# blacksnail789521/IMM-TSF

Hardware: AMD Instinct MI355X
Metric: forecast windows/sec (train fwd+bwd) on ragged 64-entity batch (higher is better)
Workload: dtype bf16

## Files before the change

### imm-tsf_amd/csrc/ttcn.hip

```cpp
#include "ttcn.hpp"
#include "../../include/immtsf.h"
#include "block_util.hpp"
#include "rowops.hpp"

int g_immtsf_ttcn_fused = 1;

namespace {

constexpr int LC = 32;

struct Dims { int P, L, F, K, NC, Fp, Kp, NCp, R; };
inline int r4(int x) { return (x + 31) / 32 * 32; }
inline Dims mk_dims(int P, int L, int te_dim, int K) {
    Dims d;
    d.P = P; d.L = L; d.F = 1 + te_dim; d.K = K; d.NC = d.F * K;
    d.Fp = r4(d.F); d.Kp = r4(K); d.NCp = r4(d.NC); d.R = P * L;
    return d;
}

__global__ __launch_bounds__(256) void build_x_kernel(Dims d, const float* __restrict__ x, const float* __restrict__ tt,
                                                       const float* ws, const float* bs, const float* __restrict__ wp,
                                                       const float* __restrict__ bp, float* __restrict__ X) {
    const long idx = (long)blockIdx.x * 256 + threadIdx.x;
    if (idx >= (long)d.R * d.Fp) return;
// ... 91 lines not shown
    const float* mp = mask + (size_t)p * d.L;
    for (int l0 = 0; l0 < d.L; l0 += LC) {
        const int lcnt = min(LC, d.L - l0);
        if (col) {
            for (int l = 0; l < lcnt; ++l) {
                const float smd = Sp[(size_t)(l0 + l) * d.NCp] * dpk;
                smt[l * d.NC + c] = smd;
                Sp[(size_t)(l0 + l) * d.NCp] = smd * (Xp[(size_t)(l0 + l) * d.Fp + fc] - ct) * mp[l0 + l];
            }
        }
        __syncthreads();
        for (int i = c; i < lcnt * d.Fp; i += nt) {
            const int l = i / d.Fp, f = i % d.Fp;
            float a = 0.f;
            if (f < d.F) for (int k = 0; k < d.K; ++k) a += smt[l * d.NC + k * d.F + f];
            dX[((size_t)p * d.L + l0 + l) * d.Fp + f] = a;
        }
        __syncthreads();
    }
}

struct Ws {
    float *X, *h1, *h2, *S, *ctr, *W1p, *b1p, *W2p, *b2p, *W3p, *b3p, *pack;
    size_t bytes;
};
Ws carve_ws(const Dims& d, void* base) {
    Carver k(base);
    Ws w;
    w.X = k.take<float>((size_t)d.R * d.Fp);
    w.h1 = k.take<float>((size_t)d.R * d.Kp);
    w.h2 = k.take<float>((size_t)d.R * d.Kp);
    w.S = k.take<float>((size_t)d.R * d.NCp);
    w.ctr = k.take<float>((size_t)d.P * (d.NC > d.F * 32 ? d.NC : d.F * 32));
    w.W1p = k.take<float>(d.Kp * d.Fp);
    w.b1p = k.take<float>(d.Kp);
    w.W2p = k.take<float>(d.Kp * d.Kp);
    w.b2p = k.take<float>(d.Kp);
    w.W3p = k.take<float>((size_t)d.NCp * d.Kp);
    w.b3p = k.take<float>(d.NCp);
    w.pack = k.take<float>(ttcn_full_pack_floats(d.F));
    w.bytes = k.bytes();
    return w;
}
struct Sc {
    float *dX, *dpool, *dz2, *dz1, *gW1p, *gb1p, *gW2p, *gb2p, *gW3p, *gb3p, *red, *slab;
    size_t bytes;
};
Sc carve_sc(const Dims& d, void* base) {
    Carver k(base);
    Sc s;
    s.dX = k.take<float>((size_t)d.R * d.Fp);
    s.dpool = k.take<float>((size_t)d.P * d.K);
    s.dz2 = k.take<float>((size_t)d.R * d.Kp);
    s.dz1 = k.take<float>((size_t)d.R * d.Kp);
    s.gW1p = k.take<float>(d.Kp * d.Fp);
    s.gb1p = k.take<float>(d.Kp);
    s.gW2p = k.take<float>(d.Kp * d.Kp);
    s.gb2p = k.take<float>(d.Kp);
    s.gW3p = k.take<float>((size_t)d.NCp * d.Kp);
    s.gb3p = k.take<float>(d.NCp);
    s.red = k.take<float>(64 * (d.NCp + 64) + 2 * 256 * d.F);
    s.slab = k.take<float>(ttcn_full_slab_floats(d.F));
    s.bytes = k.bytes();
// ... 33 lines not shown
int immtsf_patch_flatten3(const float* x, const float* tt, const float* mask, int32_t B, int32_t M, int32_t L, int32_t N, float* ox,
                          float* ott, float* omask, immtsf_stream_t stream) {
    if (!x || !tt || !mask || !ox || !ott || !omask || B < 0 || M <= 0 || L <= 0 || N <= 0) return IMMTSF_EINVAL;
    const size_t total = (size_t)B * M * L * N;
    if (total == 0) return IMMTSF_OK;
    hipLaunchKernelGGL(patch_flatten3_kernel, dim3((unsigned)((total + 255) / 256)), dim3(256), 0, static_cast<hipStream_t>(stream), x, tt, mask,
                       B, M, L, N, ox, ott, omask);
    IMMTSF_LAUNCH_CHECK();
    return IMMTSF_OK;
}

int immtsf_ttcn_forward(int32_t P, int32_t L, int32_t te_dim, int32_t ttcn_dim, int32_t precision, const float* x,
                        const float* tt, const float* mask, const immtsf_ttcn_params* p, float* out, int32_t out_ld,
                        int32_t flag_col, void* workspace, size_t workspace_bytes, immtsf_stream_t stream) {
    if (!x || !tt || !mask || !p || !out || !workspace) return IMMTSF_EINVAL;
    if (out_ld < ttcn_dim || flag_col >= out_ld || (flag_col >= 0 && flag_col < ttcn_dim)) return IMMTSF_EINVAL;
    if (bad_dims(P, L, te_dim, ttcn_dim)) return (1 + te_dim) * ttcn_dim > 1024 ? IMMTSF_EUNSUPPORTED : IMMTSF_EINVAL;
    if (P == 0) return IMMTSF_OK;
    const Dims d = mk_dims(P, L, te_dim, ttcn_dim);
    Ws w = carve_ws(d, workspace);
    if (workspace_bytes < w.bytes) return IMMTSF_EWORKSPACE;
    hipStream_t s = static_cast<hipStream_t>(stream);
    if (g_immtsf_ttcn_fused && ttcn_full_supported(precision, L, d.F, d.K))
        return launch_ttcn_full_fwd(P, L, d.F, d.K, x, tt, mask, p, w.pack, w.ctr, out, out_ld, flag_col, s);
    PackPtrs q{p->W1, p->b1, p->W2, p->b2, p->W3, p->b3, w.W1p, w.b1p, w.W2p, w.b2p, w.W3p, w.b3p};
    hipLaunchKernelGGL(pack_w_kernel, dim3(cdiv(d.NCp * d.Kp, 256)), dim3(256), 0, s, d, q);
    IMMTSF_LAUNCH_CHECK();
    const long nx = (long)d.R * d.Fp;
    hipLaunchKernelGGL(build_x_kernel, dim3((unsigned)((nx + 255) / 256)), dim3(256), 0, s, d, x, tt, p->te_scale_w, p->te_scale_b,
                       p->te_per_w, p->te_per_b, w.X);
    IMMTSF_LAUNCH_CHECK();
    {
        GemmArgs g = gemm_args(d.R, d.Kp, d.Fp, d.Fp, d.Fp, d.Kp);
        set_problem(g, 0, w.X, w.W1p, w.h1, w.b1p);
        g.act = 1;
        CHECK(immtsf_launch_gemm(GEMM_NT, precision, g, s));
    }
    {
        GemmArgs g = gemm_args(d.R, d.Kp, d.Kp, d.Kp, d.Kp, d.Kp);
        set_problem(g, 0, w.h1, w.W2p, w.h2, w.b2p);
        g.act = 1;
        CHECK(immtsf_launch_gemm(GEMM_NT, precision, g, s));
    }
    {
        GemmArgs g = gemm_args(d.R, d.NCp, d.Kp, d.Kp, d.Kp, d.NCp);
        set_problem(g, 0, w.h2, w.W3p, w.S, w.b3p);
        CHECK(immtsf_launch_gemm(GEMM_NT, precision, g, s));
    }
    const int threads = cdiv(d.NC, 64) * 64;
    hipLaunchKernelGGL(pool_fwd_kernel, dim3(P), dim3(threads), d.NC * sizeof(float), s, d, w.S, w.X, mask, p->T_bias, w.ctr, out, out_ld, flag_col);
    IMMTSF_LAUNCH_CHECK();
    return IMMTSF_OK;
}

int immtsf_ttcn_backward(int32_t P, int32_t L, int32_t te_dim, int32_t ttcn_dim, int32_t precision, const float* x,
                         const float* tt, const float* mask, const immtsf_ttcn_params* p, const float* out,
                         const float* dout, int32_t out_ld, void* workspace, size_t workspace_bytes, void* scratch,
                         size_t scratch_bytes, const immtsf_ttcn_params* gr, int32_t te_accumulate, immtsf_stream_t stream) {
    if (!tt || !mask || !p || !out || !dout || !gr || !workspace || !scratch || out_ld < ttcn_dim) return IMMTSF_EINVAL;
    if (bad_dims(P, L, te_dim, ttcn_dim)) return IMMTSF_EINVAL;
    if (P == 0) return IMMTSF_OK;
    const Dims d = mk_dims(P, L, te_dim, ttcn_dim);
    Ws w = carve_ws(d, workspace);
    Sc sc = carve_sc(d, scratch);
    if (workspace_bytes < w.bytes || scratch_bytes < sc.bytes) return IMMTSF_EWORKSPACE;
    hipStream_t s = static_cast<hipStream_t>(stream);
    if (g_immtsf_ttcn_fused && ttcn_full_supported(precision, L, d.F, d.K))
        return launch_ttcn_full_bwd(P, L, d.F, d.K, x, tt, mask, p, w.pack, w.ctr, out, dout, out_ld, sc.slab, gr,
                                    static_cast<hipStream_t>(stream), te_accumulate);
    {
        const size_t nbytes = (size_t)((char*)(sc.gb3p + d.NCp) - (char*)sc.gW1p);
        if (int rc = launch_fill(sc.gW1p, 0.f, nbytes / sizeof(float), s)) return rc;
    }
    Fork fk(s);
    {
        const int threads = cdiv(d.NC, 64) * 64;
        const size_t lds = (size_t)(d.K + LC * d.NC) * sizeof(float);
        if (lds > 160 * 1024) return IMMTSF_EUNSUPPORTED;
        hipLaunchKernelGGL(pool_bwd_kernel, dim3(P), dim3(threads), lds, s, d, w.S, w.X, mask, w.ctr, out, dout, out_ld, sc.dX, sc.dpool);
        IMMTSF_LAUNCH_CHECK();
    }
    CHECK(launch_colsum(sc.dpool, nullptr, P, nullptr, d.K, d.K, gr->T_bias, 0, sc.red, s));
    {
        GemmArgs h = gemm_args(d.NCp, d.Kp, d.R, d.NCp, d.Kp, d.Kp);
        set_problem(h, 0, w.S, w.h2, sc.gW3p, nullptr, sc.gb3p);
        h.c_prezeroed = 1;
        CHECK(immtsf_launch_gemm(GEMM_TN, precision, h, fk.fork()));
        GemmArgs g = gemm_args(d.R, d.Kp, d.NCp, d.NCp, d.Kp, d.Kp);
        set_problem(g, 0, w.S, w.W3p, sc.dz2, nullptr);
        g.relu_ref = w.h2; g.ld_ref = d.Kp;
        CHECK(immtsf_launch_gemm(GEMM_NN, precision, g, s));
// ... 31 lines not shown
```

### imm-tsf_amd/csrc/ttcn.hpp

```cpp
#pragma once
#include "common.hpp"

struct immtsf_ttcn_params;
bool ttcn_full_supported(int precision, int L, int F, int K);
size_t ttcn_full_pack_floats(int F);
size_t ttcn_full_slab_floats(int F);
int launch_ttcn_full_fwd(int P, int L, int F, int K, const float* x, const float* tt, const float* mask, const immtsf_ttcn_params* p,
                         float* pack, float* ctr, float* out, int out_ld, int flag_col, hipStream_t s);
int launch_ttcn_full_bwd(int P, int L, int F, int K, const float* x, const float* tt, const float* mask, const immtsf_ttcn_params* p,
                         const float* pack, const float* ctr, const float* out, const float* dout, int out_ld, float* slab,
                         const immtsf_ttcn_params* gr, hipStream_t s, int te_acc = 0);
```

### imm-tsf_amd/csrc/ttcn_full.hip

```cpp
#include "ttcn.hpp"
#include "../../include/immtsf.h"
#include "common.hpp"
#include <stdio.h>
#include <stdlib.h>

int g_immtsf_ttcn_bwd_grid = 0;

namespace {

typedef short s16x8 __attribute__((ext_vector_type(8)));
typedef float f32x2 __attribute__((ext_vector_type(2)));

constexpr int KP = 32;
constexpr int PT = 40;


struct FD { int P, L, F, K, NCq, dbg; };

struct Slab { int W1, b1, W2, b2, W3, b3, te, Tb, total; };
__host__ __device__ inline Slab slab_of(int F) {
    Slab s;
    int o = 0;
    s.W1 = o; o += KP * KP;
    s.b1 = o; o += KP;
    s.W2 = o; o += KP * KP;
    s.b2 = o; o += KP;
    s.W3 = o; o += F * 32 * KP;
    s.b3 = o; o += F * 32;
    s.te = o; o += 2 * KP;
    s.Tb = o; o += KP;
    s.total = o;
    return s;
}

__device__ __forceinline__ bf16x8 load8_bf16(const float* __restrict__ src) {
    const float4 a = *reinterpret_cast<const float4*>(src), b = *reinterpret_cast<const float4*>(src + 4);
    bf16x8 r;
    r[0] = (bf16_t)a.x; r[1] = (bf16_t)a.y; r[2] = (bf16_t)a.z; r[3] = (bf16_t)a.w;
    r[4] = (bf16_t)b.x; r[5] = (bf16_t)b.y; r[6] = (bf16_t)b.z; r[7] = (bf16_t)b.w;
    return r;
}
__device__ __forceinline__ float col_sum(float v) { return xor32_sum(xor16_sum(v)); }
__device__ __forceinline__ float col_max(float v) { return xor32_max(xor16_max(v)); }
__device__ __forceinline__ float row_sum16(float v) { return row16_sum(v); }
__device__ __forceinline__ bf16x8 frag_row(const bf16_t* tile, int pitch, int row0, int k0, int fr, int fq) {
    return *reinterpret_cast<const bf16x8*>(tile + (row0 + fr) * pitch + k0 + fq * 8);
}
__device__ __forceinline__ bf16x8 frag_kmajor(const bf16_t* tile, int pitch, int rbase, int kbase, int fr, int fq) {
    typedef __attribute__((address_space(3))) s16x4 lds_s16x4;
    const int q = fr >> 2, pp = fr & 3;
    const bf16_t* a0 = tile + (kbase + fq * 8 + q) * pitch + rbase + 4 * pp;
    const s16x4 lo = __builtin_amdgcn_ds_read_tr16_b64_v4i16((lds_s16x4*)(a0));
    const s16x4 hi = __builtin_amdgcn_ds_read_tr16_b64_v4i16((lds_s16x4*)(a0 + 4 * pitch));
    const s16x8 v = __builtin_shufflevector(lo, hi, 0, 1, 2, 3, 4, 5, 6, 7);
    return __builtin_bit_cast(bf16x8, v);
}
__device__ __forceinline__ f32x4 mfma(bf16x8 a, bf16x8 b, f32x4 c) { return __builtin_amdgcn_mfma_f32_16x16x32_bf16(a, b, c, 0, 0, 0); }
__device__ __forceinline__ f32x4 zero4() { return f32x4{0.f, 0.f, 0.f, 0.f}; }

struct TEp { const float *ws, *bs, *wp, *bp; };

template <int RT, bool BWD>
struct PatchIn {
    static constexpr int ROWS = RT * 16, HEAD = 3 * ROWS + (BWD ? KP : 0);
    float row, c[2];
    __device__ __forceinline__ void fetch(const FD& d, int p, const float* __restrict__ x, const float* __restrict__ tt,
                                          const float* __restrict__ mask, const float* __restrict__ ctr, const float* __restrict__ out,
                                          const float* __restrict__ dout, int out_ld) {
        const int tid = threadIdx.x;
        row = 0.f; c[0] = c[1] = 0.f;
        if (tid < 3 * ROWS) {
            const int which = tid / ROWS, l = tid % ROWS;
            if (l < d.L) row = (which == 0 ? tt : which == 1 ? x : mask)[(size_t)p * d.L + l];
        } else if (BWD && tid < HEAD) {
            const int k = tid - 3 * ROWS;
            if (k < d.K) row = out[(size_t)p * out_ld + k] > 0.f ? dout[(size_t)p * out_ld + k] : 0.f;
        }
        if (BWD) {
#pragma unroll
            for (int j = 0; j < 2; ++j) {
                const int i = tid + 256 * j;
                if (i < d.NCq) c[j] = ctr[(size_t)p * d.NCq + i];
            }
        }
    }
    __device__ __forceinline__ void park(const FD& d, float* blk) const {
        const int tid = threadIdx.x;
        if (tid < HEAD) blk[tid] = row;
        if (BWD) {
#pragma unroll
            for (int j = 0; j < 2; ++j) {
                const int i = tid + 256 * j;
                if (i < d.NCq) blk[HEAD + i] = c[j];
            }
        }
    }
};

struct XCol { float w, b; int kind; };
__device__ __forceinline__ XCol x_col(const FD& d, TEp te) {
    const int f = threadIdx.x & 31;
    XCol c{0.f, 0.f, 3};
    if (f == 0) c.kind = 0;
    else if (f == 1) { c.w = te.ws[0]; c.b = te.bs[0]; c.kind = 1; }
    else if (f < d.F) { c.w = te.wp[f - 2]; c.b = te.bp[f - 2]; c.kind = 2; }
    return c;
}

template <int RT> constexpr int xt_pitch() { return RT * 16 + 4; }
template <int RT, bool TR = false>
__device__ __forceinline__ void build_x(const FD& d, const XCol xc, const float* blk, bf16_t* Xb, float* Xf, float* Xc = nullptr) {
    const int f = threadIdx.x & 31;
#pragma unroll
    for (int j = 0; j < RT * 2; ++j) {
        const int l = (threadIdx.x >> 5) + 8 * j;
        float v = 0.f, c = 0.f, t = 0.f;
        if (l < d.L && xc.kind != 3) {
            t = blk[l];
            if (xc.kind == 0) v = blk[RT * 16 + l];
            else {
                const float ph = fmaf(xc.w, t, xc.b);
// ... 17 lines not shown
        const int rt = t >> 1, nt = t & 1;
        const f32x4 acc = mfma(frag_row(in, PT, rt * 16, 0, fr, fq), load8_bf16(W + (nt * 16 + fr) * KP + fq * 8), zero4());
        const float bias = b[nt * 16 + fr];
#pragma unroll
        for (int r = 0; r < 4; ++r) outp[(rt * 16 + fq * 4 + r) * PT + nt * 16 + fr] = (bf16_t)fmaxf(acc[r] + bias, 0.f);
    }
}

template <int RT>
__device__ __forceinline__ void mlp_layer_frag(const bf16_t* in, bf16_t* outp, const bf16x8 wf, const float bias, int wave, int fr, int fq) {
    for (int t = wave; t < RT * 2; t += 4) {
        const int rt = t >> 1, nt = t & 1;
        const f32x4 acc = mfma(frag_row(in, PT, rt * 16, 0, fr, fq), wf, zero4());
#pragma unroll
        for (int r = 0; r < 4; ++r) outp[(rt * 16 + fq * 4 + r) * PT + nt * 16 + fr] = (bf16_t)fmaxf(acc[r] + bias, 0.f);
    }
}

struct Wts { const float *W1p, *b1p, *W2p, *b2p, *W3q, *b3q; };

template <int RT, int MF>
__global__ __launch_bounds__(256) void ttcn_full_fwd_kernel(FD d, const float* __restrict__ x, const float* __restrict__ tt,
                                                             const float* __restrict__ mask, TEp te, Wts w, const bf16_t* __restrict__ W3h,
                                                             const float* __restrict__ Tb, float* __restrict__ ctr,
                                                             float* __restrict__ out, int out_ld, int flag_col) {
    extern __shared__ __attribute__((aligned(16))) unsigned char smem[];
    constexpr int ROWS = RT * 16, XP = xt_pitch<RT>();
    constexpr float LOG2E = 1.4426950408889634f;
    bf16_t* Xb = reinterpret_cast<bf16_t*>(smem);
    bf16_t* h1s = Xb + ROWS * PT;
    bf16_t* h2s = h1s + ROWS * PT;
    float* Xf = reinterpret_cast<float*>(h2s + ROWS * PT);
    float* cl = Xf + 16 * XP;
    float* pin = cl + d.NCq;
    const int tid = threadIdx.x, lane = tid & 63, wave = tid >> 6, fr = lane & 15, fq = lane >> 4;
    bf16x8 bw[MF][2];
    float b3v[MF][2];
    const int tnt = wave & 1;
    typedef PatchIn<RT, false> PI;
    PI nx;
    nx.fetch(d, blockIdx.x, x, tt, mask, nullptr, nullptr, nullptr, 0);
    const XCol xc = x_col(d, te);
    const bf16x8 mw1 = load8_bf16(w.W1p + (tnt * 16 + fr) * KP + fq * 8), mw2 = load8_bf16(w.W2p + (tnt * 16 + fr) * KP + fq * 8);
    const float mb1 = w.b1p[tnt * 16 + fr], mb2 = w.b2p[tnt * 16 + fr];
    const float tb = tid < d.K ? Tb[tid] : 0.f;
#pragma unroll
    for (int j = 0; j < MF; ++j)
#pragma unroll
        for (int half = 0; half < 2; ++half) {
            const int f = wave + 4 * j, c = f * 32 + half * 16 + fr;
            bw[j][half] = bf16x8{0, 0, 0, 0, 0, 0, 0, 0};
            b3v[j][half] = 0.f;
            if (f < d.F) { bw[j][half] = *reinterpret_cast<const bf16x8*>(W3h + (size_t)c * KP + fq * 8); b3v[j][half] = w.b3q[c] * LOG2E; }
        }
    nx.park(d, pin);
    __syncthreads();
    int it = 0;
    for (int p = blockIdx.x; p < d.P; p += gridDim.x, ++it) {
    const float* cur = pin + (it & 1) * PI::HEAD;
    const int pn = p + gridDim.x;
    if (pn < d.P) nx.fetch(d, pn, x, tt, mask, nullptr, nullptr, nullptr, 0);
    build_x<RT, true>(d, xc, cur, Xb, Xf);
    __syncthreads();
    mlp_layer_frag<RT>(Xb, h1s, mw1, mb1, wave, fr, fq);
    __syncthreads();
    mlp_layer_frag<RT>(h1s, h2s, mw2, mb2, wave, fr, fq);
    __syncthreads();
    bf16x8 a[RT];
    bool on[RT][4];
    float cval[RT][4];
#pragma unroll
    for (int rt = 0; rt < RT; ++rt) {
        a[rt] = frag_row(h2s, PT, rt * 16, 0, fr, fq);
        const f32x4 m4 = *reinterpret_cast<const f32x4*>(cur + 2 * ROWS + rt * 16 + fq * 4);
#pragma unroll
        for (int r = 0; r < 4; ++r) {
            on[rt][r] = m4[r] != 0.f;
            cval[rt][r] = rt * 16 + fq * 4 + r < d.L ? -1e8f * LOG2E : -INFINITY;
        }
    }
#pragma unroll
    for (int j = 0; j < MF; ++j) {
        const int f = wave + 4 * j;
        if (f < d.F) {
// ... 23 lines not shown
                            m = fmaxf(m, v[rt][h][e]);
                        }
                }
                m = col_max(m);
                f32x2 s2{0.f, 0.f}, p2{0.f, 0.f};
#pragma unroll
                for (int rt = 0; rt < RT; ++rt)
#pragma unroll
                    for (int h = 0; h < 2; ++h) {
                        v[rt][h] -= m;
                        v[rt][h][0] = __builtin_amdgcn_exp2f(v[rt][h][0]);
                        v[rt][h][1] = __builtin_amdgcn_exp2f(v[rt][h][1]);
                        s2 += v[rt][h];
                        p2 += v[rt][h] * xf[rt][h];
                    }
                const float acc = col_sum(p2[0] + p2[1]) * __builtin_amdgcn_rcpf(col_sum(s2[0] + s2[1]));
                if (fq == 0) {
                    cl[c] = acc;
                    ctr[(size_t)p * d.NCq + c] = acc;
                }
            }
        }
    }
    if (pn < d.P) nx.park(d, pin + ((it + 1) & 1) * PI::HEAD);
    __syncthreads();
    if (tid < d.K) {
        float s = tb;
        for (int f = 0; f < d.F; ++f) s += cl[f * 32 + tid];
        out[(size_t)p * out_ld + tid] = fmaxf(s, 0.f);
    }
    if (flag_col >= 0 && wave == 1) {
        float any = lane < d.L ? cur[2 * ROWS + lane] : 0.f;
        any = wave_sum(any);
        if (lane == 0) out[(size_t)p * out_ld + flag_col] = any > 0.f ? 1.f : 0.f;
    }
    __syncthreads();
    }
}

struct WtsT { const bf16_t *W3T , *W2T , *W1T , *W3h ; };

template <int RT, int MF>
__global__ __launch_bounds__(256) __attribute__((amdgpu_waves_per_eu(RT == 2 ? 2 : 1))) void ttcn_full_bwd_kernel(FD d, const float* __restrict__ x, const float* __restrict__ tt,
                                                             const float* __restrict__ mask, TEp te, Wts w, WtsT wt,
                                                             const float* __restrict__ ctr, const float* __restrict__ out,
                                                             const float* __restrict__ dout, int out_ld, float* __restrict__ slab) {
    extern __shared__ __attribute__((aligned(16))) unsigned char smem[];
    constexpr int ROWS = RT * 16, PTT = ROWS + 8, XP = xt_pitch<RT>();
    constexpr float LOG2E = 1.4426950408889634f;
    bf16_t* Xb = reinterpret_cast<bf16_t*>(smem);
    bf16_t* h1s = Xb + ROWS * PT;
    bf16_t* h2s = h1s + ROWS * PT;
    bf16_t* dz2s = h2s + ROWS * PT;
    bf16_t* dz1s = h2s;
    bf16_t* dST = dz2s + ROWS * PT;
    float* Xf = reinterpret_cast<float*>(dST + d.NCq * PTT);
    float* Xc = Xf + 16 * XP;
    typedef PatchIn<RT, true> PI;
    const int PIN = PI::HEAD + d.NCq;
    float* pin = Xc + 16 * XP;
    bf16_t* W3s = reinterpret_cast<bf16_t*>(pin + 2 * PIN);
    bf16_t* W1s = W3s + d.NCq * PT;
    bf16_t* W2s = W1s + KP * PT;
    float* b3s = reinterpret_cast<float*>(W2s + KP * PT);
    const int tid = threadIdx.x, lane = tid & 63, wave = tid >> 6, fr = lane & 15, fq = lane >> 4;
    const Slab sl = slab_of(d.F);
    PI nx;
    nx.fetch(d, blockIdx.x, x, tt, mask, ctr, out, dout, out_ld);
    const XCol xc = x_col(d, te);
    for (int i = tid; i < d.NCq * 4; i += 256) {
        const int c = i >> 2, q = i & 3;
        *reinterpret_cast<bf16x8*>(W3s + c * PT + q * 8) = *reinterpret_cast<const bf16x8*>(wt.W3h + (size_t)c * KP + q * 8);
    }
    for (int i = tid; i < d.NCq; i += 256) b3s[i] = w.b3q[i] * LOG2E;
    if (tid < 2 * KP * 4) {
        const int which = tid >> 7, r = (tid >> 2) & 31, q = tid & 3;
        *reinterpret_cast<bf16x8*>((which ? W2s : W1s) + r * PT + q * 8) = load8_bf16((which ? w.W2p : w.W1p) + r * KP + q * 8);
    }

    f32x4 accW3[MF][2][2];
    f32x2 accB3[MF][2];
#pragma unroll
    for (int j = 0; j < MF; ++j)
#pragma unroll
        for (int half = 0; half < 2; ++half) {
            accW3[j][half][0] = zero4(); accW3[j][half][1] = zero4();
            accB3[j][half] = f32x2{0.f, 0.f};
        }
    const int tnt = wave & 1, tmt = wave >> 1;
    const float mb1 = w.b1p[tnt * 16 + fr], mb2 = w.b2p[tnt * 16 + fr];
    f32x4 accW2 = zero4(), accW1 = zero4();
    float sb2 = 0.f, sb1 = 0.f;
    float accT = 0.f;
    float te_w = 0.f, te_b = 0.f;
    f32x2 tpw[MF], tpb[MF];
#pragma unroll
    for (int j = 0; j < MF; ++j) tpw[j] = tpb[j] = f32x2{0.f, 0.f};

    nx.park(d, pin);
    __syncthreads();
    int it = 0;
    for (int p = blockIdx.x; p < d.P; p += gridDim.x, ++it) {
        const float* cur = pin + (it & 1) * PIN;
        const float *dp = cur + 3 * ROWS, *cts = cur + PI::HEAD;
        const int pn = p + gridDim.x;
        if (pn < d.P) nx.fetch(d, pn, x, tt, mask, ctr, out, dout, out_ld);
        build_x<RT, true>(d, xc, cur, Xb, Xf, Xc);
        __syncthreads();
        if (tid >= 128 && tid < 128 + KP) accT += dp[tid - 128];
        mlp_layer_frag<RT>(Xb, h1s, frag_row(W1s, PT, tnt * 16, 0, fr, fq), mb1, wave, fr, fq);
        __syncthreads();
        mlp_layer_frag<RT>(h1s, h2s, frag_row(W2s, PT, tnt * 16, 0, fr, fq), mb2, wave, fr, fq);
        __syncthreads();
        bf16x8 a[RT];
        bool on[RT][4];
        float cval[RT][4], anyf = 0.f;
        f32x4 t4[RT];
#pragma unroll
        for (int rt = 0; rt < RT; ++rt) {
            a[rt] = frag_row(h2s, PT, rt * 16, 0, fr, fq);
            t4[rt] = *reinterpret_cast<const f32x4*>(cur + rt * 16 + fq * 4);
            const f32x4 m4 = *reinterpret_cast<const f32x4*>(cur + 2 * ROWS + rt * 16 + fq * 4);
#pragma unroll
            for (int r = 0; r < 4; ++r) {
                on[rt][r] = m4[r] != 0.f;
                cval[rt][r] = rt * 16 + fq * 4 + r < d.L ? -1e8f * LOG2E : -INFINITY;
                anyf += on[rt][r] ? 1.f : 0.f;
            }
        }
// ... 108 lines not shown
                const int o = (rt * 16 + fq * 4 + r) * PT + tnt * 16 + fr;
                const float g = (float)h1s[o] > 0.f ? acc[r] : 0.f;
                dz1s[o] = (bf16_t)g;
                sb1 += g;
            }
        }
        __syncthreads();
        if (wave < 2) {
#pragma unroll
            for (int kk = 0; kk < ROWS; kk += 32)
                accW1 = mfma(frag_kmajor(dz1s, PT, wave * 16, kk, fr, fq), frag_kmajor(Xb, PT, 0, kk, fr, fq), accW1);
        }
        for (int rt = (RT == 2 ? wave - 2 : wave); rt >= 0 && rt < RT; rt += 4) {
            const f32x4 acc = mfma(frag_row(dz1s, PT, rt * 16, 0, fr, fq), frag_kmajor(W1s, PT, 0, 0, fr, fq), zero4());
            const f32x4 c4 = *reinterpret_cast<const f32x4*>(Xc + fr * XP + rt * 16 + fq * 4);
            const f32x4 tr = *reinterpret_cast<const f32x4*>(cur + rt * 16 + fq * 4);
#pragma unroll
            for (int r = 0; r < 4; ++r) {
                const float g = acc[r] * c4[r];
                te_w = fmaf(g, tr[r], te_w);
                te_b += g;
            }
        }
        if (pn < d.P) nx.park(d, pin + ((it + 1) & 1) * PIN);
        __syncthreads();
    }

    float* my = slab + (size_t)blockIdx.x * sl.total;
#pragma unroll
    for (int j = 0; j < MF; ++j) {
        const int f = wave + 4 * j;
        if (f < d.F) {
#pragma unroll
            for (int half = 0; half < 2; ++half) {
#pragma unroll
                for (int nt = 0; nt < 2; ++nt)
#pragma unroll
                    for (int r = 0; r < 4; ++r)
                        my[sl.W3 + (size_t)(f * 32 + half * 16 + fq * 4 + r) * KP + nt * 16 + fr] = accW3[j][half][nt][r];
                const float b3sum = col_sum(accB3[j][half][0] + accB3[j][half][1]);
                if (fq == 0) my[sl.b3 + f * 32 + half * 16 + fr] = b3sum;
            }
        }
    }
#pragma unroll
    for (int r = 0; r < 4; ++r) {
        my[sl.W2 + (tmt * 16 + fq * 4 + r) * KP + tnt * 16 + fr] = accW2[r];
        if (wave < 2) my[sl.W1 + (wave * 16 + fq * 4 + r) * KP + fr] = accW1[r];
    }
    if (tid >= 128 && tid < 128 + KP) my[sl.Tb + tid - 128] = accT;
    float* tes = pin;
    if (tid < 4 * KP) tes[tid] = 0.f;
    __syncthreads();
#pragma unroll
    for (int j = 0; j < MF; ++j) {
        const int f = wave + 4 * j;
        const float sw = col_sum(row_sum16(tpw[j][0] + tpw[j][1])), sb = col_sum(row_sum16(tpb[j][0] + tpb[j][1]));
        if (lane == 0 && f >= 1 && f < d.F) {
            atomicAdd(tes + f, sw);
            atomicAdd(tes + KP + f, sb);
        }
    }
    te_w = col_sum(te_w);
    te_b = col_sum(te_b);
    sb2 = col_sum(sb2);
    sb1 = col_sum(sb1);
    if (fq == 0) {
        if (RT == 4 || wave >= 2) {
            atomicAdd(tes + fr, te_w);
            atomicAdd(tes + KP + fr, te_b);
        }
        atomicAdd(tes + 2 * KP + tnt * 16 + fr, sb2);
        atomicAdd(tes + 3 * KP + tnt * 16 + fr, sb1);
    }
    __syncthreads();
    if (tid < 2 * KP) my[sl.te + tid] = tes[tid];
    else if (tid < 3 * KP) my[sl.b2 + tid - 2 * KP] = tes[tid];
    else if (tid < 4 * KP) my[sl.b1 + tid - 3 * KP] = tes[tid];
}

struct PackIn { const float *W1, *b1, *W2, *b2, *W3, *b3; };
__global__ __launch_bounds__(256) void ttcn_pack_kernel(int F, int K, PackIn q, float* W1p, float* b1p, float* W2p, float* b2p,
                                                         float* W3q, float* b3q, bf16_t* W3T, bf16_t* W2T, bf16_t* W1T, bf16_t* W3h) {
    const int i = blockIdx.x * 256 + threadIdx.x, NCq = F * 32;
    if (i < KP * KP) {
        const int r = i >> 5, c = i & 31;
        const float v1 = (r < K && c < F) ? q.W1[r * F + c] : 0.f, v2 = (r < K && c < K) ? q.W2[r * K + c] : 0.f;
        W1p[i] = v1;
        W2p[i] = v2;
        W1T[c * KP + r] = (bf16_t)v1;
        W2T[c * KP + r] = (bf16_t)v2;
    }
    if (i < KP) { b1p[i] = i < K ? q.b1[i] : 0.f; b2p[i] = i < K ? q.b2[i] : 0.f; }
    if (i < NCq * KP) {
        const int c = i >> 5, kk = i & 31, f = c >> 5, k = c & 31;
        const float v = (k < K && kk < K) ? q.W3[(size_t)(k * F + f) * K + kk] : 0.f;
        W3q[i] = v;
        W3T[(size_t)kk * NCq + c] = (bf16_t)v;
        W3h[i] = (bf16_t)v;
    }
    if (i < NCq) { const int f = i >> 5, k = i & 31; b3q[i] = k < K ? q.b3[k * F + f] : 0.f; }
}

struct UnpackOut { float *W1, *b1, *W2, *b2, *W3, *b3, *ws, *bs, *wp, *bp, *Tb; };
__global__ __launch_bounds__(256) void ttcn_unpack_kernel(int F, int K, const float* __restrict__ slab, int nslab, UnpackOut g, int te_acc) {
    __shared__ float red[8][33];
// ... 10 lines not shown
    else if ((i -= n) < K) { dst = g.b1 + i; off = sl.b1 + i; }
    else if ((i -= K) < K) { dst = g.b2 + i; off = sl.b2 + i; }
    else if ((i -= K) < K) { dst = g.Tb + i; off = sl.Tb + i; }
    else if ((i -= K) < 1) { dst = g.ws; off = sl.te + 1; acc = te_acc != 0; }
    else if ((i -= 1) < 1) { dst = g.bs; off = sl.te + KP + 1; acc = te_acc != 0; }
    else if ((i -= 1) < F - 2) { dst = g.wp + i; off = sl.te + 2 + i; acc = te_acc != 0; }
    else if ((i -= F - 2) < F - 2) { dst = g.bp + i; off = sl.te + KP + 2 + i; acc = te_acc != 0; }
    float s = 0.f;
    if (dst) {
#pragma unroll 8
        for (int w = part; w < nslab; w += 8) s += slab[(size_t)w * sl.total + off];
    }
    red[part][slot] = s;
    __syncthreads();
    if (part == 0 && dst) {
#pragma unroll
        for (int q = 1; q < 8; ++q) s += red[q][slot];
        *dst = (acc ? *dst : 0.f) + s;
    }
}
inline int ttcn_unpack_outputs(int F, int K) { return K * F + K * K + F * K * K + F * K + 3 * K + 2 + 2 * (F - 2); }
constexpr int kMaxBwdGrid = 512;

size_t fwd_lds(int RT, int NCq) { return (size_t)RT * 16 * PT * 2 * 3 + (size_t)16 * (RT * 16 + 4) * 4 + (size_t)NCq * 4 + (size_t)2 * 3 * RT * 16 * 4 + 64; }
size_t bwd_lds(int RT, int NCq) {
    const size_t ROWS = RT * 16;
    return ROWS * PT * 2 * 4 + (size_t)NCq * (ROWS + 8) * 2 + 16 * (ROWS + 4) * 4 * 2 + 2 * (3 * ROWS + KP + (size_t)NCq) * 4 + (size_t)(NCq + 2 * KP) * PT * 2 + (size_t)NCq * 4;
}

struct PackPtrs { float *W1p, *b1p, *W2p, *b2p, *W3q, *b3q; bf16_t *W3T, *W2T, *W1T, *W3h; };
PackPtrs pack_ptrs(float* base, int F) {
    PackPtrs q;
    float* o = base;
    q.W1p = o; o += KP * KP;
    q.W2p = o; o += KP * KP;
    q.b1p = o; o += KP;
    q.b2p = o; o += KP;
    q.W3q = o; o += (size_t)F * 32 * KP;
    q.b3q = o; o += F * 32;
    q.W3T = reinterpret_cast<bf16_t*>(o); o += (size_t)F * 32 * KP / 2;
    q.W2T = reinterpret_cast<bf16_t*>(o); o += KP * KP / 2;
    q.W1T = reinterpret_cast<bf16_t*>(o); o += KP * KP / 2;
    q.W3h = reinterpret_cast<bf16_t*>(o);
    return q;
}

}

bool ttcn_full_supported(int precision, int L, int F, int K) {
    return precision == 1 && K >= 1 && K <= 32 && F >= 2 && F <= 16 && L >= 1 && L <= 64;
}
size_t ttcn_full_pack_floats(int F) { return (size_t)2 * KP * KP + 2 * KP + (size_t)F * 32 * KP + F * 32 + (size_t)F * 32 * KP + KP * KP + 64; }
size_t ttcn_full_slab_floats(int F) { return (size_t)kMaxBwdGrid * slab_of(F).total; }

int launch_ttcn_full_fwd(int P, int L, int F, int K, const float* x, const float* tt, const float* mask, const immtsf_ttcn_params* p,
                         float* pack, float* ctr, float* out, int out_ld, int flag_col, hipStream_t s) {
    const FD d{P, L, F, K, F * 32};
    const PackPtrs q = pack_ptrs(pack, F);
    hipLaunchKernelGGL(ttcn_pack_kernel, dim3(cdiv(F * 32 * KP, 256)), dim3(256), 0, s, F, K, PackIn{p->W1, p->b1, p->W2, p->b2, p->W3, p->b3},
                       q.W1p, q.b1p, q.W2p, q.b2p, q.W3q, q.b3q, q.W3T, q.W2T, q.W1T, q.W3h);
    IMMTSF_LAUNCH_CHECK();
    const TEp te{p->te_scale_w, p->te_scale_b, p->te_per_w, p->te_per_b};
    const Wts w{q.W1p, q.b1p, q.W2p, q.b2p, q.W3q, q.b3q};
    const int mf = (F + 3) / 4;
#define TTCN_FWD(RT, MF)                                                                                                                     \
    hipLaunchKernelGGL((ttcn_full_fwd_kernel<RT, MF>), dim3(P < 2048 ? P : 2048), dim3(256), fwd_lds(RT, d.NCq), s, d, x, tt, mask, te, w, q.W3h, p->T_bias, ctr, \
                       out, out_ld, flag_col)
    if (L <= 32) {
        if (mf == 1) TTCN_FWD(2, 1); else if (mf == 2) TTCN_FWD(2, 2); else if (mf == 3) TTCN_FWD(2, 3); else TTCN_FWD(2, 4);
    } else {
        if (mf == 1) TTCN_FWD(4, 1); else if (mf == 2) TTCN_FWD(4, 2); else if (mf == 3) TTCN_FWD(4, 3); else TTCN_FWD(4, 4);
    }
#undef TTCN_FWD
    IMMTSF_LAUNCH_CHECK();
    return IMMTSF_OK;
}

int launch_ttcn_full_bwd(int P, int L, int F, int K, const float* x, const float* tt, const float* mask, const immtsf_ttcn_params* p,
                         const float* pack, const float* ctr, const float* out, const float* dout, int out_ld, float* slab,
                         const immtsf_ttcn_params* gr, hipStream_t s, int te_acc) {
    const FD d{P, L, F, K, F * 32, 0};
    const PackPtrs q = pack_ptrs(const_cast<float*>(pack), F);
    const TEp te{p->te_scale_w, p->te_scale_b, p->te_per_w, p->te_per_b};
    const Wts w{q.W1p, q.b1p, q.W2p, q.b2p, q.W3q, q.b3q};
    const WtsT wt{q.W3T, q.W2T, q.W1T, q.W3h};
    const int genv = g_immtsf_ttcn_bwd_grid;
    int gmax = genv > 0 ? genv : (L <= 32 ? (P >= 8192 ? 512 : 384) : 224);
    gmax = gmax > kMaxBwdGrid ? kMaxBwdGrid : gmax;
    const int grid = P < gmax ? P : gmax;
    const size_t lds = bwd_lds(L <= 32 ? 2 : 4, d.NCq);
    const int mf = (F + 3) / 4;
#define TTCN_BWD(RT, MF)                                                                                                                  \
    do {                                                                                                                                  \
        if (lds > 64 * 1024)                                                                                                              \
            (void)hipFuncSetAttribute(reinterpret_cast<const void*>(ttcn_full_bwd_kernel<RT, MF>), hipFuncAttributeMaxDynamicSharedMemorySize, \
                                      (int)lds);                                                                                          \
        hipLaunchKernelGGL((ttcn_full_bwd_kernel<RT, MF>), dim3(grid), dim3(256), lds, s, d, x, tt, mask, te, w, wt, ctr, out, dout, out_ld, \
                           slab);                                                                                                         \
    } while (0)
    if (L <= 32) {
        if (mf == 1) TTCN_BWD(2, 1); else if (mf == 2) TTCN_BWD(2, 2); else if (mf == 3) TTCN_BWD(2, 3); else TTCN_BWD(2, 4);
    } else {
        if (mf == 1) TTCN_BWD(4, 1); else if (mf == 2) TTCN_BWD(4, 2); else if (mf == 3) TTCN_BWD(4, 3); else TTCN_BWD(4, 4);
    }
#undef TTCN_BWD
    IMMTSF_LAUNCH_CHECK();
    hipLaunchKernelGGL(ttcn_unpack_kernel, dim3(cdiv(ttcn_unpack_outputs(F, K), 32)), dim3(256), 0, s, F, K, slab, grid,
                       UnpackOut{gr->W1, gr->b1, gr->W2, gr->b2, gr->W3, gr->b3, gr->te_scale_w, gr->te_scale_b, gr->te_per_w, gr->te_per_b,
                                 gr->T_bias}, te_acc);
    IMMTSF_LAUNCH_CHECK();
    return IMMTSF_OK;
}
```

Baseline: 157,500.

## Partition TTCN patches into live and empty lists, fast-path fully-masked patches

Adds an ordering pass, fused into the weight-pack kernel plus an optional scatter kernel for large P, that classifies each patch as live or empty (all-zero mask) and writes a compacted index list. The forward and backward fused kernels walk this list, skipping the MLP and GEMM work for empty patches. Forward computes only the mean-based outputs for them; backward handles them in a separate cheap loop that accumulates only the time-embedding gradients. It also swaps some shared-memory atomics for per-wave staging and a deterministic sum. This costs an extra mask scan and more complex control flow, and could pay off on ragged batches with many empty patches.

```diff
diff --git a/imm-tsf_amd/csrc/ttcn.hip b/imm-tsf_amd/csrc/ttcn.hip
--- a/imm-tsf_amd/csrc/ttcn.hip
+++ b/imm-tsf_amd/csrc/ttcn.hip
@@ -137,6 +137,7 @@
 
 struct Ws {
     float *X, *h1, *h2, *S, *ctr, *W1p, *b1p, *W2p, *b2p, *W3p, *b3p, *pack;
+    int* order;
     size_t bytes;
 };
 Ws carve_ws(const Dims& d, void* base) {
@@ -154,6 +155,7 @@
     w.W3p = k.take<float>((size_t)d.NCp * d.Kp);
     w.b3p = k.take<float>(d.NCp);
     w.pack = k.take<float>(ttcn_full_pack_floats(d.F));
+    w.order = k.take<int>(ttcn_full_order_ints(d.P));
     w.bytes = k.bytes();
     return w;
 }
@@ -233,7 +235,7 @@
     if (workspace_bytes < w.bytes) return IMMTSF_EWORKSPACE;
     hipStream_t s = static_cast<hipStream_t>(stream);
     if (g_immtsf_ttcn_fused && ttcn_full_supported(precision, L, d.F, d.K))
-        return launch_ttcn_full_fwd(P, L, d.F, d.K, x, tt, mask, p, w.pack, w.ctr, out, out_ld, flag_col, s);
+        return launch_ttcn_full_fwd(P, L, d.F, d.K, x, tt, mask, p, w.pack, w.order, w.ctr, out, out_ld, flag_col, s);
     PackPtrs q{p->W1, p->b1, p->W2, p->b2, p->W3, p->b3, w.W1p, w.b1p, w.W2p, w.b2p, w.W3p, w.b3p};
     hipLaunchKernelGGL(pack_w_kernel, dim3(cdiv(d.NCp * d.Kp, 256)), dim3(256), 0, s, d, q);
     IMMTSF_LAUNCH_CHECK();
@@ -277,7 +279,7 @@
     if (workspace_bytes < w.bytes || scratch_bytes < sc.bytes) return IMMTSF_EWORKSPACE;
     hipStream_t s = static_cast<hipStream_t>(stream);
     if (g_immtsf_ttcn_fused && ttcn_full_supported(precision, L, d.F, d.K))
-        return launch_ttcn_full_bwd(P, L, d.F, d.K, x, tt, mask, p, w.pack, w.ctr, out, dout, out_ld, sc.slab, gr,
+        return launch_ttcn_full_bwd(P, L, d.F, d.K, x, tt, mask, p, w.pack, w.order, w.ctr, out, dout, out_ld, sc.slab, gr,
                                     static_cast<hipStream_t>(stream), te_accumulate);
     {
         const size_t nbytes = (size_t)((char*)(sc.gb3p + d.NCp) - (char*)sc.gW1p);
diff --git a/imm-tsf_amd/csrc/ttcn.hpp b/imm-tsf_amd/csrc/ttcn.hpp
--- a/imm-tsf_amd/csrc/ttcn.hpp
+++ b/imm-tsf_amd/csrc/ttcn.hpp
@@ -5,8 +5,9 @@
 bool ttcn_full_supported(int precision, int L, int F, int K);
 size_t ttcn_full_pack_floats(int F);
 size_t ttcn_full_slab_floats(int F);
+size_t ttcn_full_order_ints(int P);
 int launch_ttcn_full_fwd(int P, int L, int F, int K, const float* x, const float* tt, const float* mask, const immtsf_ttcn_params* p,
-                         float* pack, float* ctr, float* out, int out_ld, int flag_col, hipStream_t s);
+                         float* pack, int* order, float* ctr, float* out, int out_ld, int flag_col, hipStream_t s);
 int launch_ttcn_full_bwd(int P, int L, int F, int K, const float* x, const float* tt, const float* mask, const immtsf_ttcn_params* p,
-                         const float* pack, const float* ctr, const float* out, const float* dout, int out_ld, float* slab,
-                         const immtsf_ttcn_params* gr, hipStream_t s, int te_acc = 0);
+                         const float* pack, const int* order, const float* ctr, const float* out, const float* dout, int out_ld,
+                         float* slab, const immtsf_ttcn_params* gr, hipStream_t s, int te_acc = 0);
diff --git a/imm-tsf_amd/csrc/ttcn_full.hip b/imm-tsf_amd/csrc/ttcn_full.hip
--- a/imm-tsf_amd/csrc/ttcn_full.hip
+++ b/imm-tsf_amd/csrc/ttcn_full.hip
@@ -16,6 +16,9 @@
 
 
 struct FD { int P, L, F, K, NCq, dbg; };
+
+constexpr int kOrdLive = 0, kOrdList = 4;
+constexpr int kOrdOneWg = 8192, kOrdChunk = 1024;
 
 struct Slab { int W1, b1, W2, b2, W3, b3, te, Tb, total; };
 __host__ __device__ inline Slab slab_of(int F) {
@@ -59,6 +62,16 @@
 __device__ __forceinline__ f32x4 zero4() { return f32x4{0.f, 0.f, 0.f, 0.f}; }
 
 struct TEp { const float *ws, *bs, *wp, *bp; };
+__device__ __forceinline__ void stage_te(const FD& d, TEp te, float* tes) {
+    const int f = threadIdx.x;
+    if (f < 16) {
+        float w = 0.f, b = 0.f;
+        if (f == 1) { w = te.ws[0]; b = te.bs[0]; }
+        else if (f >= 2 && f < d.F) { w = te.wp[f - 2]; b = te.bp[f - 2]; }
+        tes[f] = w;
+        tes[16 + f] = b;
+    }
+}
 
 template <int RT, bool BWD>
 struct PatchIn {
@@ -97,6 +110,23 @@
     }
 };
 
+template <int RT>
+__device__ __forceinline__ float fetch_empty(const FD& d, int p, const float* __restrict__ tt, const float* __restrict__ out,
+                                             const float* __restrict__ dout, int out_ld) {
+    constexpr int ROWS = RT * 16;
+    const int tid = threadIdx.x, k = tid - 3 * ROWS;
+    float v = 0.f;
+    if (tid < ROWS) { if (tid < d.L) v = tt[(size_t)p * d.L + tid]; }
+    else if (k >= 0 && k < d.K) v = out[(size_t)p * out_ld + k] > 0.f ? dout[(size_t)p * out_ld + k] : 0.f;
+    return v;
+}
+template <int RT>
+__device__ __forceinline__ void park_empty(float* blk, float v) {
+    constexpr int ROWS = RT * 16;
+    const int tid = threadIdx.x;
+    if (tid < ROWS || (tid >= 3 * ROWS && tid < 3 * ROWS + KP)) blk[tid] = v;
+}
+
 struct XCol { float w, b; int kind; };
 __device__ __forceinline__ XCol x_col(const FD& d, TEp te) {
     const int f = threadIdx.x & 31;
@@ -160,8 +190,8 @@
 template <int RT, int MF>
 __global__ __launch_bounds__(256) void ttcn_full_fwd_kernel(FD d, const float* __restrict__ x, const float* __restrict__ tt,
                                                              const float* __restrict__ mask, TEp te, Wts w, const bf16_t* __restrict__ W3h,
-                                                             const float* __restrict__ Tb, float* __restrict__ ctr,
-                                                             float* __restrict__ out, int out_ld, int flag_col) {
+                                                             const float* __restrict__ Tb, const int* __restrict__ ord,
+                                                             float* __restrict__ ctr, float* __restrict__ out, int out_ld, int flag_col) {
     extern __shared__ __attribute__((aligned(16))) unsigned char smem[];
     constexpr int ROWS = RT * 16, XP = xt_pitch<RT>();
     constexpr float LOG2E = 1.4426950408889634f;
@@ -171,14 +201,20 @@
     float* Xf = reinterpret_cast<float*>(h2s + ROWS * PT);
     float* cl = Xf + 16 * XP;
     float* pin = cl + d.NCq;
+    float* tes = pin + 2 * 3 * ROWS;
     const int tid = threadIdx.x, lane = tid & 63, wave = tid >> 6, fr = lane & 15, fq = lane >> 4;
+    const int n_live = ord[kOrdLive];
+    const int* __restrict__ list = ord + kOrdList;
+    const int grid = gridDim.x;
+    int p = list[blockIdx.x], pn = blockIdx.x + grid < d.P ? list[blockIdx.x + grid] : -1;
     bf16x8 bw[MF][2];
     float b3v[MF][2];
     const int tnt = wave & 1;
     typedef PatchIn<RT, false> PI;
     PI nx;
-    nx.fetch(d, blockIdx.x, x, tt, mask, nullptr, nullptr, nullptr, 0);
+    nx.fetch(d, p, x, tt, mask, nullptr, nullptr, nullptr, 0);
     const XCol xc = x_col(d, te);
+    stage_te(d, te, tes);
     const bf16x8 mw1 = load8_bf16(w.W1p + (tnt * 16 + fr) * KP + fq * 8), mw2 = load8_bf16(w.W2p + (tnt * 16 + fr) * KP + fq * 8);
     const float mb1 = w.b1p[tnt * 16 + fr], mb2 = w.b2p[tnt * 16 + fr];
     const float tb = tid < d.K ? Tb[tid] : 0.f;
@@ -194,10 +230,29 @@
     nx.park(d, pin);
     __syncthreads();
     int it = 0;
-    for (int p = blockIdx.x; p < d.P; p += gridDim.x, ++it) {
+    for (int i = blockIdx.x; i < d.P; i += grid, ++it) {
     const float* cur = pin + (it & 1) * PI::HEAD;
-    const int pn = p + gridDim.x;
-    if (pn < d.P) nx.fetch(d, pn, x, tt, mask, nullptr, nullptr, nullptr, 0);
+    const int pnn = i + 2 * grid < d.P ? list[i + 2 * grid] : -1;
+    if (pn >= 0) nx.fetch(d, pn, x, tt, mask, nullptr, nullptr, nullptr, 0);
+    if (i >= n_live) {
+        const float invL = __builtin_amdgcn_rcpf((float)d.L);
+#pragma unroll
+        for (int j = 0; j < MF; ++j) {
+            const int f = wave + 4 * j;
+            if (f < d.F) {
+                float v = 0.f;
+                if (lane < d.L) {
+                    const float ph = fmaf(tes[f], cur[lane], tes[16 + f]);
+                    v = f == 0 ? cur[ROWS + lane] : f == 1 ? ph : __sinf(ph);
+                }
+                const float mean = wave_sum(v) * invL;
+                if (lane < 32) {
+                    cl[f * 32 + lane] = mean;
+                    ctr[(size_t)p * d.NCq + f * 32 + lane] = mean;
+                }
+            }
+        }
+    } else {
     build_x<RT, true>(d, xc, cur, Xb, Xf);
     __syncthreads();
     mlp_layer_frag<RT>(Xb, h1s, mw1, mb1, wave, fr, fq);
@@ -267,7 +322,8 @@
             }
         }
     }
-    if (pn < d.P) nx.park(d, pin + ((it + 1) & 1) * PI::HEAD);
+    }
+    if (pn >= 0) nx.park(d, pin + ((it + 1) & 1) * PI::HEAD);
     __syncthreads();
     if (tid < d.K) {
         float s = tb;
@@ -280,6 +336,8 @@
         if (lane == 0) out[(size_t)p * out_ld + flag_col] = any > 0.f ? 1.f : 0.f;
     }
     __syncthreads();
+    p = pn;
+    pn = pnn;
     }
 }
 
@@ -289,7 +347,8 @@
 __global__ __launch_bounds__(256) __attribute__((amdgpu_waves_per_eu(RT == 2 ? 2 : 1))) void ttcn_full_bwd_kernel(FD d, const float* __restrict__ x, const float* __restrict__ tt,
                                                              const float* __restrict__ mask, TEp te, Wts w, WtsT wt,
                                                              const float* __restrict__ ctr, const float* __restrict__ out,
-                                                             const float* __restrict__ dout, int out_ld, float* __restrict__ slab) {
+                                                             const float* __restrict__ dout, int out_ld, const int* __restrict__ ord,
+                                                             float* __restrict__ slab) {
     extern __shared__ __attribute__((aligned(16))) unsigned char smem[];
     constexpr int ROWS = RT * 16, PTT = ROWS + 8, XP = xt_pitch<RT>();
     constexpr float LOG2E = 1.4426950408889634f;
@@ -308,11 +367,19 @@
     bf16_t* W1s = W3s + d.NCq * PT;
     bf16_t* W2s = W1s + KP * PT;
     float* b3s = reinterpret_cast<float*>(W2s + KP * PT);
+    float* tep = b3s + d.NCq;
     const int tid = threadIdx.x, lane = tid & 63, wave = tid >> 6, fr = lane & 15, fq = lane >> 4;
     const Slab sl = slab_of(d.F);
+    const int n_live = ord[kOrdLive], n_empty = d.P - n_live, grid = gridDim.x;
+    const int* __restrict__ list = ord + kOrdList;
+    int pn = (int)blockIdx.x + grid < n_live ? list[blockIdx.x + grid] : -1;
+    const int e0 = grid - 1 - (int)blockIdx.x;
+    int pe = e0 < n_empty ? list[n_live + e0] : -1, pen = e0 + grid < n_empty ? list[n_live + e0 + grid] : -1;
     PI nx;
-    nx.fetch(d, blockIdx.x, x, tt, mask, ctr, out, dout, out_ld);
+    if ((int)blockIdx.x < n_live) nx.fetch(d, list[blockIdx.x], x, tt, mask, ctr, out, dout, out_ld);
+    float erow = pe >= 0 ? fetch_empty<RT>(d, pe, tt, out, dout, out_ld) : 0.f;
     const XCol xc = x_col(d, te);
+    stage_te(d, te, tep);
     for (int i = tid; i < d.NCq * 4; i += 256) {
         const int c = i >> 2, q = i & 3;
         *reinterpret_cast<bf16x8*>(W3s + c * PT + q * 8) = *reinterpret_cast<const bf16x8*>(wt.W3h + (size_t)c * KP + q * 8);
@@ -342,14 +409,14 @@
 #pragma unroll
     for (int j = 0; j < MF; ++j) tpw[j] = tpb[j] = f32x2{0.f, 0.f};
 
-    nx.park(d, pin);
+    if ((int)blockIdx.x < n_live) nx.park(d, pin);
     __syncthreads();
     int it = 0;
-    for (int p = blockIdx.x; p < d.P; p += gridDim.x, ++it) {
+    for (int i = blockIdx.x; i < n_live; i += grid, ++it) {
         const float* cur = pin + (it & 1) * PIN;
         const float *dp = cur + 3 * ROWS, *cts = cur + PI::HEAD;
-        const int pn = p + gridDim.x;
-        if (pn < d.P) nx.fetch(d, pn, x, tt, mask, ctr, out, dout, out_ld);
+        const int pnn = i + 2 * grid < n_live ? list[i + 2 * grid] : -1;
+        if (pn >= 0) nx.fetch(d, pn, x, tt, mask, ctr, out, dout, out_ld);
         build_x<RT, true>(d, xc, cur, Xb, Xf, Xc);
         __syncthreads();
         if (tid >= 128 && tid < 128 + KP) accT += dp[tid - 128];
@@ -504,8 +571,39 @@
                 te_b += g;
             }
         }
-        if (pn < d.P) nx.park(d, pin + ((it + 1) & 1) * PIN);
+        if (pn >= 0) nx.park(d, pin + ((it + 1) & 1) * PIN);
         __syncthreads();
+        pn = pnn;
+    }
+
+    if (pe >= 0) {
+        park_empty<RT>(pin, erow);
+        __syncthreads();
+        const float invL = __builtin_amdgcn_rcpf((float)d.L);
+        int eit = 0;
+        for (int e = e0; e < n_empty; e += grid, ++eit) {
+            const float* cur = pin + (eit & 1) * PIN;
+            const float* dp = cur + 3 * ROWS;
+            const int penn = e + 2 * grid < n_empty ? list[n_live + e + 2 * grid] : -1;
+            if (pen >= 0) erow = fetch_empty<RT>(d, pen, tt, out, dout, out_ld);
+            if (tid >= 128 && tid < 128 + KP) accT += dp[tid - 128];
+            const float s = wave_sum(lane < KP ? dp[lane] : 0.f) * invL;
+            if (lane < d.L) {
+                const float t = cur[lane];
+#pragma unroll
+                for (int j = 0; j < MF; ++j) {
+                    const int f = wave + 4 * j;
+                    if (f >= 1 && f < d.F) {
+                        const float g = f == 1 ? s : s * __cosf(fmaf(tep[f], t, tep[16 + f]));
+                        tpb[j][0] += g;
+                        tpw[j][0] = fmaf(g, t, tpw[j][0]);
+                    }
+                }
+            }
+            if (pen >= 0) park_empty<RT>(pin + ((eit + 1) & 1) * PIN, erow);
+            __syncthreads();
+            pen = penn;
+        }
     }
 
     float* my = slab + (size_t)blockIdx.x * sl.total;
@@ -539,31 +637,129 @@
         const int f = wave + 4 * j;
         const float sw = col_sum(row_sum16(tpw[j][0] + tpw[j][1])), sb = col_sum(row_sum16(tpb[j][0] + tpb[j][1]));
         if (lane == 0 && f >= 1 && f < d.F) {
-            atomicAdd(tes + f, sw);
-            atomicAdd(tes + KP + f, sb);
+            tes[f] = sw;
+            tes[KP + f] = sb;
         }
     }
     te_w = col_sum(te_w);
     te_b = col_sum(te_b);
     sb2 = col_sum(sb2);
     sb1 = col_sum(sb1);
+    float* mlp = tes + 4 * KP;
     if (fq == 0) {
-        if (RT == 4 || wave >= 2) {
-            atomicAdd(tes + fr, te_w);
-            atomicAdd(tes + KP + fr, te_b);
-        }
+        mlp[wave * KP + fr] = (RT == 4 || wave >= 2) ? te_w : 0.f;
+        mlp[wave * KP + 16 + fr] = (RT == 4 || wave >= 2) ? te_b : 0.f;
         atomicAdd(tes + 2 * KP + tnt * 16 + fr, sb2);
         atomicAdd(tes + 3 * KP + tnt * 16 + fr, sb1);
     }
     __syncthreads();
+    if (tid < 2 * KP && (tid & 31) < 16) {
+        const int o = (tid >> 5) * 16 + (tid & 31);
+        tes[tid] += ((mlp[o] + mlp[KP + o]) + mlp[2 * KP + o]) + mlp[3 * KP + o];
+    }
     if (tid < 2 * KP) my[sl.te + tid] = tes[tid];
     else if (tid < 3 * KP) my[sl.b2 + tid - 2 * KP] = tes[tid];
     else if (tid < 4 * KP) my[sl.b1 + tid - 3 * KP] = tes[tid];
 }
 
+struct OrdPtrs { int *base, *loc, *cnt; };
+__device__ __forceinline__ void ttcn_order_chunk(const float* __restrict__ mask, int L, int p0, int np, bool whole, OrdPtrs o) {
+    __shared__ unsigned char flg[kOrdOneWg];
+    __shared__ int wtot[4];
+    const int tid = threadIdx.x, lane = tid & 63, wave = tid >> 6;
+    for (int i = tid; i < np; i += 256) flg[i] = 0;
+    __syncthreads();
+    const float* m = mask + (size_t)p0 * L;
+    const int n = np * L;
+    const int head = min(n, (int)(((16 - (reinterpret_cast<uintptr_t>(m) & 15)) & 15) >> 2)), nvec = (n - head) >> 2;
+    const float4* mv = reinterpret_cast<const float4*>(m + head);
+    const int tail = head + nvec * 4 + tid;
+    if (tid < head && m[tid] != 0.f) flg[tid / L] = 1;
+    if (tail < n && m[tail] != 0.f) flg[tail / L] = 1;
+    constexpr int U = 8;
+    for (int base = 0; base < nvec; base += 256 * U) {
+        float4 v[U];
+#pragma unroll
+        for (int u = 0; u < U; ++u) {
+            const int i = base + u * 256 + tid;
+            v[u] = i < nvec ? mv[i] : float4{0.f, 0.f, 0.f, 0.f};
+        }
+#pragma unroll
+        for (int u = 0; u < U; ++u) {
+            if (v[u].x != 0.f || v[u].y != 0.f || v[u].z != 0.f || v[u].w != 0.f) {
+                const int e = head + 4 * (base + u * 256 + tid);
+                int pp = e / L, r = e - pp * L;
+                const float c[4] = {v[u].x, v[u].y, v[u].z, v[u].w};
+#pragma unroll
+                for (int j = 0; j < 4; ++j) {
+                    if (c[j] != 0.f) flg[pp] = 1;
+                    if (++r == L) { r = 0; ++pp; }
+                }
+            }
+        }
+    }
+    __syncthreads();
+    const int per = (np + 255) / 256, a = min(np, tid * per), b = min(np, a + per);
+    int cnt = 0;
+    for (int i = a; i < b; ++i) cnt += flg[i];
+    int incl = cnt;
+#pragma unroll
+    for (int s = 1; s < 64; s <<= 1) {
+        const int up = __shfl_up(incl, s);
+        if (lane >= s) incl += up;
+    }
+    if (lane == 63) wtot[wave] = incl;
+    __syncthreads();
+    int before = incl - cnt, total = 0;
+#pragma unroll
+    for (int w = 0; w < 4; ++w) {
+        if (w < wave) before += wtot[w];
+        total += wtot[w];
+    }
+    for (int i = a; i < b; ++i) {
+        const bool live = flg[i] != 0;
+        const int rank = live ? before : i - before;
+        if (whole) o.base[kOrdList + (live ? rank : total + rank)] = i;
+        else o.loc[p0 + i] = live ? rank : -1 - rank;
+        before += live ? 1 : 0;
+    }
+    if (tid == 0) {
+        if (whole) o.base[kOrdLive] = total;
+        else o.cnt[p0 / kOrdChunk] = total;
+    }
+}
+__global__ __launch_bounds__(256) void ttcn_order_scatter_kernel(int P, OrdPtrs o) {
+    __shared__ int sums[2];
+    const int tid = threadIdx.x, p = blockIdx.x * 256 + tid, chunk = blockIdx.x * 256 / kOrdChunk, nchunk = (P + kOrdChunk - 1) / kOrdChunk;
+    if (tid < 2) sums[tid] = 0;
+    __syncthreads();
+    int front = 0, all = 0;
+    for (int c = tid; c < nchunk; c += 256) {
+        const int v = o.cnt[c];
+        all += v;
+        if (c < chunk) front += v;
+    }
+    if (front) atomicAdd(&sums[0], front);
+    if (all) atomicAdd(&sums[1], all);
+    __syncthreads();
+    front = sums[0];
+    all = sums[1];
+    if (p < P) {
+        const int l = o.loc[p];
+        o.base[kOrdList + (l >= 0 ? front + l : all + (chunk * kOrdChunk - front) + (-1 - l))] = p;
+    }
+    if (p == 0) o.base[kOrdLive] = all;
+}
+
 struct PackIn { const float *W1, *b1, *W2, *b2, *W3, *b3; };
 __global__ __launch_bounds__(256) void ttcn_pack_kernel(int F, int K, PackIn q, float* W1p, float* b1p, float* W2p, float* b2p,
-                                                         float* W3q, float* b3q, bf16_t* W3T, bf16_t* W2T, bf16_t* W1T, bf16_t* W3h) {
+                                                         float* W3q, float* b3q, bf16_t* W3T, bf16_t* W2T, bf16_t* W1T, bf16_t* W3h,
+                                                         int npack, const float* __restrict__ mask, int P, int L, OrdPtrs ord) {
+    if ((int)blockIdx.x >= npack) {
+        const int p0 = P < kOrdOneWg ? 0 : ((int)blockIdx.x - npack) * kOrdChunk;
+        ttcn_order_chunk(mask, L, p0, P < kOrdOneWg ? P : min(kOrdChunk, P - p0), P < kOrdOneWg, ord);
+        return;
+    }
     const int i = blockIdx.x * 256 + threadIdx.x, NCq = F * 32;
     if (i < KP * KP) {
         const int r = i >> 5, c = i & 31;
@@ -620,10 +816,10 @@
 inline int ttcn_unpack_outputs(int F, int K) { return K * F + K * K + F * K * K + F * K + 3 * K + 2 + 2 * (F - 2); }
 constexpr int kMaxBwdGrid = 512;
 
-size_t fwd_lds(int RT, int NCq) { return (size_t)RT * 16 * PT * 2 * 3 + (size_t)16 * (RT * 16 + 4) * 4 + (size_t)NCq * 4 + (size_t)2 * 3 * RT * 16 * 4 + 64; }
+size_t fwd_lds(int RT, int NCq) { return (size_t)RT * 16 * PT * 2 * 3 + (size_t)16 * (RT * 16 + 4) * 4 + (size_t)NCq * 4 + (size_t)2 * 3 * RT * 16 * 4 + 32 * 4 + 64; }
 size_t bwd_lds(int RT, int NCq) {
     const size_t ROWS = RT * 16;
-    return ROWS * PT * 2 * 4 + (size_t)NCq * (ROWS + 8) * 2 + 16 * (ROWS + 4) * 4 * 2 + 2 * (3 * ROWS + KP + (size_t)NCq) * 4 + (size_t)(NCq + 2 * KP) * PT * 2 + (size_t)NCq * 4;
+    return ROWS * PT * 2 * 4 + (size_t)NCq * (ROWS + 8) * 2 + 16 * (ROWS + 4) * 4 * 2 + 2 * (3 * ROWS + KP + (size_t)NCq) * 4 + (size_t)(NCq + 2 * KP) * PT * 2 + (size_t)NCq * 4 + 32 * 4;
 }
 
 struct PackPtrs { float *W1p, *b1p, *W2p, *b2p, *W3q, *b3q; bf16_t *W3T, *W2T, *W1T, *W3h; };
@@ -650,19 +846,26 @@
 }
 size_t ttcn_full_pack_floats(int F) { return (size_t)2 * KP * KP + 2 * KP + (size_t)F * 32 * KP + F * 32 + (size_t)F * 32 * KP + KP * KP + 64; }
 size_t ttcn_full_slab_floats(int F) { return (size_t)kMaxBwdGrid * slab_of(F).total; }
+size_t ttcn_full_order_ints(int P) { return (size_t)kOrdList + P + (P >= kOrdOneWg ? (size_t)P + (P + kOrdChunk - 1) / kOrdChunk : 0); }
 
 int launch_ttcn_full_fwd(int P, int L, int F, int K, const float* x, const float* tt, const float* mask, const immtsf_ttcn_params* p,
-                         float* pack, float* ctr, float* out, int out_ld, int flag_col, hipStream_t s) {
+                         float* pack, int* order, float* ctr, float* out, int out_ld, int flag_col, hipStream_t s) {
     const FD d{P, L, F, K, F * 32};
     const PackPtrs q = pack_ptrs(pack, F);
-    hipLaunchKernelGGL(ttcn_pack_kernel, dim3(cdiv(F * 32 * KP, 256)), dim3(256), 0, s, F, K, PackIn{p->W1, p->b1, p->W2, p->b2, p->W3, p->b3},
-                       q.W1p, q.b1p, q.W2p, q.b2p, q.W3q, q.b3q, q.W3T, q.W2T, q.W1T, q.W3h);
+    const int npack = cdiv(F * 32 * KP, 256), nord = P < kOrdOneWg ? 1 : cdiv(P, kOrdChunk);
+    const OrdPtrs op{order, order + kOrdList + P, order + kOrdList + 2 * (size_t)P};
+    hipLaunchKernelGGL(ttcn_pack_kernel, dim3(npack + nord), dim3(256), 0, s, F, K, PackIn{p->W1, p->b1, p->W2, p->b2, p->W3, p->b3},
+                       q.W1p, q.b1p, q.W2p, q.b2p, q.W3q, q.b3q, q.W3T, q.W2T, q.W1T, q.W3h, npack, mask, P, L, op);
     IMMTSF_LAUNCH_CHECK();
+    if (P >= kOrdOneWg) {
+        hipLaunchKernelGGL(ttcn_order_scatter_kernel, dim3(cdiv(P, 256)), dim3(256), 0, s, P, op);
+        IMMTSF_LAUNCH_CHECK();
+    }
     const TEp te{p->te_scale_w, p->te_scale_b, p->te_per_w, p->te_per_b};
     const Wts w{q.W1p, q.b1p, q.W2p, q.b2p, q.W3q, q.b3q};
     const int mf = (F + 3) / 4;
 #define TTCN_FWD(RT, MF)                                                                                                                     \
-    hipLaunchKernelGGL((ttcn_full_fwd_kernel<RT, MF>), dim3(P < 2048 ? P : 2048), dim3(256), fwd_lds(RT, d.NCq), s, d, x, tt, mask, te, w, q.W3h, p->T_bias, ctr, \
+    hipLaunchKernelGGL((ttcn_full_fwd_kernel<RT, MF>), dim3(P < 2048 ? P : 2048), dim3(256), fwd_lds(RT, d.NCq), s, d, x, tt, mask, te, w, q.W3h, p->T_bias, order, ctr, \
                        out, out_ld, flag_col)
     if (L <= 32) {
         if (mf == 1) TTCN_FWD(2, 1); else if (mf == 2) TTCN_FWD(2, 2); else if (mf == 3) TTCN_FWD(2, 3); else TTCN_FWD(2, 4);
@@ -675,8 +878,8 @@
 }
 
 int launch_ttcn_full_bwd(int P, int L, int F, int K, const float* x, const float* tt, const float* mask, const immtsf_ttcn_params* p,
-                         const float* pack, const float* ctr, const float* out, const float* dout, int out_ld, float* slab,
-                         const immtsf_ttcn_params* gr, hipStream_t s, int te_acc) {
+                         const float* pack, const int* order, const float* ctr, const float* out, const float* dout, int out_ld,
+                         float* slab, const immtsf_ttcn_params* gr, hipStream_t s, int te_acc) {
     const FD d{P, L, F, K, F * 32, 0};
     const PackPtrs q = pack_ptrs(const_cast<float*>(pack), F);
     const TEp te{p->te_scale_w, p->te_scale_b, p->te_per_w, p->te_per_b};
@@ -694,7 +897,7 @@
             (void)hipFuncSetAttribute(reinterpret_cast<const void*>(ttcn_full_bwd_kernel<RT, MF>), hipFuncAttributeMaxDynamicSharedMemorySize, \
                                       (int)lds);                                                                                          \
         hipLaunchKernelGGL((ttcn_full_bwd_kernel<RT, MF>), dim3(grid), dim3(256), lds, s, d, x, tt, mask, te, w, wt, ctr, out, dout, out_ld, \
-                           slab);                                                                                                         \
+                           order, slab);                                                                                                         \
     } while (0)
     if (L <= 32) {
         if (mf == 1) TTCN_BWD(2, 1); else if (mf == 2) TTCN_BWD(2, 2); else if (mf == 3) TTCN_BWD(2, 3); else TTCN_BWD(2, 4);
```

After: 155,800. 1.0% lower.
